# sailordiary/m3f.pytorch

Hardware: AMD Instinct MI355X
Metric: clips/sec (300-frame A+V, fwd+bwd) (higher is better)
Workload: dtype f32 (fp32-accurate products, fp32 accumulate: GEMMs as fp16x3 -- two fp16 terms per scaled operand, three MFMAs, error vs fp64 no larger than an fp32 GEMM's; the forward and backward recurrences at H=512 and H=256 as fp16x3 too (h is bounded; the backward producers split their values under a power-o

## Files before the change

include/m3t_hip.h:

```cpp
#ifndef M3T_HIP_H
#define M3T_HIP_H

#include <stddef.h>
#include <stdint.h>

#ifdef __cplusplus
extern "C" {
#endif

#define M3T_EINVAL 10001
#define M3T_MAX_SCANS 8
#define M3T_ESPIN 10002
#define M3T_SCAN_NO_PERSIST 1
#define M3T_SCAN_WHH 8
#define M3T_SCAN_FP32 4
#define M3T_SCAN_FAULT 16
#define M3T_SCAN_WIDE 32
#define M3T_BF16 2
#define M3T_GEMM_BACKGROUND 1
#define M3T_GEMM_BF16 2
#define M3T_GEMM_HIGH 256
#define M3T_GEMM_F16X3 1024
#define M3T_GEMM_BESIDE_SCAN 512
#define M3T_GEMM_EXCLUSIVE 8
// ... 105 lines not shown
    unsigned long long* amax;
    const float* wfrag;
} m3t_gru_bwd_desc;

size_t m3t_gru_bwd_prepare_floats(int H);
int m3t_gru_bwd_prepare(const float* const* w, int n, int H, int whh_direct, float* const* out, void* stream);

int m3t_gru_scan_workgroups(int n_scans, int H, int B, int T, int flags, int backward);
int m3t_gru_persist_count(void);
int m3t_gru_poll_error(void);
int m3t_gru_error_reset(void);
int m3t_gru_error_defer(int on);
int m3t_gru_inject_error(void* stream);
int m3t_gru_persist_owner(void);
int m3t_gru_scan_arena(void* arena, size_t bytes);
int m3t_gru_scan_arena_reset(void* arena);
int m3t_gru_scan_progress(unsigned* counters, int n_marks, const int* time_bounds, unsigned* need);
int m3t_gru_scan_progress_reset(unsigned* counters);
int m3t_gru_scan_progress_ok(int n_scans, int H, int B, int T, int flags, int backward);
int m3t_stream_wait_progress(const unsigned* counter, unsigned need, void* stream);
int m3t_gru_scan_after(void* event);
int m3t_gru_scan_events(void* start, void* end);
int m3t_gru_persist_profile(unsigned long long* out6);

int m3t_gru_scan_bwd(const m3t_gru_bwd_desc* scans, int n_scans, int B, int T,
                     float* ws, size_t ws_bytes, int flags, void* stream);

int m3t_att_fuse_fwd(const float* s_v, const float* s_a, const float* x_v, const float* x_a,
                     float* f, int rows, int D, void* stream);
int m3t_att_fuse_bwd(const float* df, const float* s_v, const float* s_a,
                     const float* x_v, const float* x_a,
                     float* ds_v, float* ds_a, float* dx_v, float* dx_a,
                     int rows, int D, void* stream);

int m3t_va_loss(const float* y_hat, int rows, int C, int iv, int ia,
                const float* valence, const float* arousal,
                const int64_t* class_expr, const uint8_t* expr_valid, int n_expr,
                float w_v, float w_a, float expr_w, int use_mse,
                float* out_scalars, float* dy, float* ws, size_t ws_bytes, void* stream);
size_t m3t_va_loss_ws_bytes(int rows);

size_t m3t_bn_cl_ws_bytes(size_t M, int C);
int m3t_bn_pool_cl_fwd(const float* x, size_t P, int H, int W, int C, int k, const float* gamma, const float* beta, float* run_mean, float* run_var,
                       float momentum, float eps, int training, float* yp, unsigned char* win, float* save_mean, float* save_invstd, float* ws,
                       size_t ws_bytes, void* stream);
int m3t_bn_pool_cl_bwd(const float* dyp, const float* x, const float* yp, const unsigned char* win, const float* gamma, const float* save_mean,
                       const float* save_invstd, size_t P, int H, int W, int C, int k, int training, float* dx, float* dgamma, float* dbeta,
                       float* dx_colsum, float* ws, size_t ws_bytes, void* stream);
int m3t_bn_cl_fwd(const float* x, size_t M, int C, const float* gamma, const float* beta, float* run_mean, float* run_var, float momentum,
                  float eps, int training, int relu, float* y, float* save_mean, float* save_invstd, float* ws, size_t ws_bytes, void* stream);
int m3t_bn_cl_bwd(const float* dy, const float* x, const float* y, const float* gamma, const float* save_mean, const float* save_invstd, size_t M,
                  int C, int training, int relu, float* dx, float* dgamma, float* dbeta, float* dx_colsum, float* ws, size_t ws_bytes, void* stream);
int m3t_pool_cl_fwd(const float* x, size_t P, int H, int W, int C, int kh, int kw, int sh, int sw, int ph, int pw, float* y, unsigned char* win,
                    void* stream);
int m3t_pool_cl_bwd(const float* dy, const unsigned char* win, size_t P, int H, int W, int C, int kh, int kw, int sh, int sw, int ph, int pw,
                    float* dx, void* stream);

int m3t_bn_add_relu_cl_fwd(const float* x, const float* shortcut, size_t M, int C, const float* gamma, const float* beta, float* run_mean,
                           float* run_var, float momentum, float eps, int training, float* y, float* save_mean, float* save_invstd, float* ws,
                           size_t ws_bytes, void* stream);
int m3t_bn_add_relu_cl_bwd(const float* dy, const float* x, const float* y, const float* gamma, const float* save_mean, const float* save_invstd,
                           size_t M, int C, int training, float* dx, float* ds, float* dgamma, float* dbeta, float* dx_colsum, float* ws,
                           size_t ws_bytes, void* stream);
int m3t_mean_cl_fwd(const float* x, size_t P, int HW, int C, float* y, void* stream);
int m3t_mean_cl_bwd(const float* dy, size_t P, int HW, int C, float* dx, void* stream);

// ... 260 lines not shown
```

m3f.pytorch_amd/csrc/fuse_loss.hip:

```cpp
#include "gru_common.h"
#include <cmath>
#include <cstdlib>
#include <mutex>

namespace {

__device__ __forceinline__ void fuse_weights(float sv, float sa, float& hv, float& ha, float& w0, float& w1) {
    hv = 1.f / (1.f + expf(-sv));
    ha = 1.f / (1.f + expf(-sa));
    const float m = fmaxf(hv, ha);
    const float ev = expf(hv - m), ea = expf(ha - m);
    const float inv = 1.f / (ev + ea);
    w0 = ev * inv;
    w1 = ea * inv;
}

__device__ __forceinline__ float mix2(float w0, float v, float w1, float a) { return fmaf(w0, v, w1 * a); }

__global__ __launch_bounds__(256) void att_fuse_fwd_kernel(const float* __restrict__ s_v, const float* __restrict__ s_a,
                                                           const float* __restrict__ x_v, const float* __restrict__ x_a,
                                                           float* __restrict__ f, int rows, int D, int vec) {
    const int lane = threadIdx.x & 63;
    const int row = blockIdx.x * 4 + (threadIdx.x >> 6);
    if (row >= rows) return;
// ... 23 lines not shown
    if (row >= rows) return;
    float hv, ha, w0, w1;
    fuse_weights(s_v[row], s_a[row], hv, ha, w0, w1);
    const size_t base = (size_t)row * D;
    float d0 = 0.f, d1 = 0.f;
    if (vec) {
        const float4* pg = reinterpret_cast<const float4*>(df + base);
        const float4* pv = reinterpret_cast<const float4*>(x_v + base);
        const float4* pa = reinterpret_cast<const float4*>(x_a + base);
        float4* qv = reinterpret_cast<float4*>(dx_v + base);
        float4* qa = reinterpret_cast<float4*>(dx_a + base);
        for (int i = lane; i < (D >> 2); i += 64) {
            const float4 g = pg[i], v = pv[i], a = pa[i];
            d0 += g.x * v.x + g.y * v.y + g.z * v.z + g.w * v.w;
            d1 += g.x * a.x + g.y * a.y + g.z * a.z + g.w * a.w;
            qv[i] = make_float4(w0 * g.x, w0 * g.y, w0 * g.z, w0 * g.w);
            qa[i] = make_float4(w1 * g.x, w1 * g.y, w1 * g.z, w1 * g.w);
        }
    } else {
        for (int i = lane; i < D; i += 64) {
            const float g = df[base + i];
            d0 += g * x_v[base + i];
            d1 += g * x_a[base + i];
            dx_v[base + i] = w0 * g;
            dx_a[base + i] = w1 * g;
        }
    }
    d0 = wave_sum(d0);
    d1 = wave_sum(d1);
    if (lane == 0) {
        const float dot = w0 * d0 + w1 * d1;
        ds_v[row] = w0 * (d0 - dot) * hv * (1.f - hv);
        ds_a[row] = w1 * (d1 - dot) * ha * (1.f - ha);
    }
}

__device__ __forceinline__ double wave_sum_d(double v) {
#pragma unroll
    for (int o = 32; o > 0; o >>= 1) v += __shfl_xor(v, o, 64);
    return v;
}
__device__ __forceinline__ double block_sum_d(double v, double* red) {
    const int lane = threadIdx.x & 63, w = threadIdx.x >> 6, nw = (blockDim.x + 63) >> 6;
    v = wave_sum_d(v);
    __syncthreads();
    if (lane == 0) red[w] = v;
    __syncthreads();
    double r = 0.0;
    for (int i = 0; i < nw; ++i) r += red[i];
    return r;
}

struct VaTerm { double mx, mt, ccc, mse, c1, c2, c3; };

__device__ __forceinline__ VaTerm va_term(double mx, double mt, double cov, double vsum, double mse, double invn, double nm1) {
    VaTerm s;
    const double den = vsum + (mx - mt) * (mx - mt);
    const double q = 2.0 * cov / (den * den);
    s.mx = mx; s.mt = mt; s.mse = mse;
    s.ccc = 2.0 * cov / den;
    s.c1 = 2.0 * invn / den;
    s.c2 = q * 2.0 * nm1;
    s.c3 = q * 2.0 * (mx - mt) * invn;
    return s;
}

// ... 387 lines not shown
extern "C" int m3t_sgd_step(float* p, const float* g, float* buf, size_t n, float lr, float momentum, float weight_decay,
                            int step, const float* guard, void* stream) {
    if (n == 0) return 0;
    if (!p || !g || !buf || step < 1) return M3T_EINVAL;
    int blocks = (int)((n + 255) / 256);
    if (blocks > 4096) blocks = 4096;
    sgd_kernel<<<blocks, 256, 0, (hipStream_t)stream>>>(p, g, buf, n, lr, momentum, weight_decay, step == 1, guard);
    M3T_LAUNCH_CHECK();
    return 0;
}

extern "C" int m3t_att_fuse_fwd(const float* s_v, const float* s_a, const float* x_v, const float* x_a, float* f,
                                int rows, int D, void* stream) {
    if (rows <= 0 || D <= 0) return 0;
    if (!s_v || !s_a || !x_v || !x_a || !f) return M3T_EINVAL;
    const int vec = (D % 4 == 0) && (((uintptr_t)x_v | (uintptr_t)x_a | (uintptr_t)f) % 16 == 0);
    att_fuse_fwd_kernel<<<cdiv(rows, 4), 256, 0, (hipStream_t)stream>>>(s_v, s_a, x_v, x_a, f, rows, D, vec);
    M3T_LAUNCH_CHECK();
    return 0;
}

extern "C" int m3t_att_fuse_bwd(const float* df, const float* s_v, const float* s_a, const float* x_v, const float* x_a,
                                float* ds_v, float* ds_a, float* dx_v, float* dx_a, int rows, int D, void* stream) {
    if (rows <= 0 || D <= 0) return 0;
    if (!df || !s_v || !s_a || !x_v || !x_a || !ds_v || !ds_a || !dx_v || !dx_a) return M3T_EINVAL;
    const int vec = (D % 4 == 0) &&
                    (((uintptr_t)x_v | (uintptr_t)x_a | (uintptr_t)df | (uintptr_t)dx_v | (uintptr_t)dx_a) % 16 == 0);
    att_fuse_bwd_kernel<<<cdiv(rows, 4), 256, 0, (hipStream_t)stream>>>(df, s_v, s_a, x_v, x_a, ds_v, ds_a, dx_v, dx_a,
                                                                         rows, D, vec);
    M3T_LAUNCH_CHECK();
    return 0;
}

extern "C" size_t m3t_va_loss_ws_bytes(int rows) { return rows > 0 ? (size_t)cdiv(rows, LB) * 16 * sizeof(double) : 0; }

extern "C" int m3t_va_loss(const float* y_hat, int rows, int C, int iv, int ia, const float* valence,
                           const float* arousal, const int64_t* class_expr, const uint8_t* expr_valid, int n_expr,
                           float w_v, float w_a, float expr_w, int use_mse, float* out_scalars, float* dy,
                           float* ws, size_t ws_bytes, void* stream) {
    if (rows <= 0 || C <= 0 || iv < 0 || ia < 0 || iv >= C || ia >= C || n_expr > C) return M3T_EINVAL;
    if (!y_hat || !valence || !arousal || !out_scalars || !dy) return M3T_EINVAL;
    if (n_expr > 0 && (!class_expr || !expr_valid)) return M3T_EINVAL;
    static const bool fused_on = !(getenv("M3T_VA_LOSS_FUSED") && getenv("M3T_VA_LOSS_FUSED")[0] == '0');
    const bool ws_ok = ws && ((uintptr_t)ws % 8) == 0 && ws_bytes >= m3t_va_loss_ws_bytes(rows);
    double* part = reinterpret_cast<double*>(ws);
    if (rows > 1024 && ws_ok && cdiv(rows, LB) <= 128 && fused_on) {
        VaSync* sync = va_sync_words();
        if (sync) {
            const int nb = cdiv(rows, LB);
            va_loss_fused_kernel<<<nb, LB, 0, (hipStream_t)stream>>>(y_hat, rows, C, iv, ia, valence, arousal, class_expr, expr_valid, n_expr, w_v,
                                                                     w_a, expr_w, use_mse, part, sync, 1 << 22, out_scalars, dy);
            M3T_LAUNCH_CHECK();
            return 0;
        }
    }
    if (rows > 1024 && ws_ok) {
        const int nb = cdiv(rows, LB);
        double* partA = part;
        double* partB = part + (size_t)nb * 8;
        hipStream_t s = (hipStream_t)stream;
        va_loss_sums_kernel<<<nb, LB, 0, s>>>(y_hat, rows, C, iv, ia, valence, arousal, class_expr, expr_valid, n_expr, partA);
        va_loss_moments_kernel<<<nb, LB, 0, s>>>(y_hat, rows, C, iv, ia, valence, arousal, partA, partB);
        va_loss_grad_kernel<<<nb, LB, 0, s>>>(y_hat, rows, C, iv, ia, valence, arousal, class_expr, expr_valid, n_expr, w_v, w_a,
                                             expr_w, use_mse, partA, partB, out_scalars, dy);
        M3T_LAUNCH_CHECK();
        return 0;
// ... 52 lines not shown
```

m3f.pytorch_amd/m3t/_lib.py:

```python
import ctypes as C
import os

_HERE = os.path.dirname(os.path.abspath(__file__))
LIB_PATH = os.environ.get("M3T_LIB_PATH") or os.path.join(os.path.dirname(_HERE), "lib", "libm3t_hip.so")
CSRC_DIR = os.path.join(os.path.dirname(_HERE), "csrc")

M3T_EINVAL = 10001
M3T_ESPIN = 10002
M3T_SCAN_NO_PERSIST = 1
M3T_BF16 = 2
M3T_GEMM_BESIDE_SCAN = 512
M3T_GEMM_F16X3 = 1024
M3T_GEMM_HIGH = 256
M3T_GEMM_EXCLUSIVE = 8
M3T_CONV_IMAGES = 4096
M3T_SCAN_FP32 = 4
M3T_SCAN_WHH = 8
M3T_SCAN_FAULT = 16
M3T_SCAN_WIDE = 32
M3T_MAX_SCANS = 8
M3T_JPEG_TRUNC, M3T_JPEG_CODE, M3T_JPEG_RST, M3T_JPEG_EXTRA = 1, 2, 4, 8

_f = C.c_void_p
_i = C.c_int
# ... 43 lines not shown
    "m3t_sgemm_bimg": [_i, _i, _i, _f, _i, _f, _f, _i, _f, _i, _i, _f, _z, _f, _f, _s],
    "m3t_sgemm_ring": [_i, _i, _i, _i, _i, _f, _i, _f, _i, _f, _i, _f, _i, _i, _i, _i, _i, _i, _f, _z, _i, _f, _f, _i, _s],
    "m3t_conv3d_taps_pre": [_f, _f, _f] + [_i] * 16 + [_f, _f, _f, _z, _f, _s],
    "m3t_conv3d_fwd_taps": [_f, _f, _f, _f] + [_i] * 15 + [_f, _f, _f, _z, _f, _s],
    "m3t_conv3d_fwd_taps4": [_f, _f, _f, _f] + [_i] * 14 + [_f, _f, _f, _z, _f, _s],
    "m3t_planes_to_cl4": [_f, _f, _i, _i, C.c_longlong, _s],
    "m3t_conv3d_wgrad_taps": [_f, _f, _f] + [_i] * 16 + [_f, _f, _f, _z, _s],
    "m3t_amax_out": [C.c_void_p],
    "m3t_colsum": [_f, _i, _i, _i, _f, _i, _f, _z, _s],
    "m3t_transpose": [_f, _i, _i, _i, _f, _i, _s],
    "m3t_relu_bwd": [_f, _f, _z, _s],
    "m3t_gru_scan_fwd": [C.POINTER(GruFwdDesc), _i, _i, _i, _f, _z, _i, _s],
    "m3t_gru_scan_bwd": [C.POINTER(GruBwdDesc), _i, _i, _i, _f, _z, _i, _s],
    "m3t_gru_bwd_prepare_floats": [_i],
    "m3t_gru_bwd_prepare": [C.POINTER(C.c_void_p), _i, _i, _i, C.POINTER(C.c_void_p), _s],
    "m3t_gru_persist_count": [],
    "m3t_gru_scan_workgroups": [_i, _i, _i, _i, _i, _i],
    "m3t_gru_poll_error": [],
    "m3t_gru_error_reset": [],
    "m3t_gru_error_defer": [_i],
    "m3t_gru_inject_error": [_s],
    "m3t_gru_persist_owner": [],
    "m3t_gru_scan_arena": [C.c_void_p, _z],
    "m3t_gru_scan_arena_reset": [C.c_void_p],
    "m3t_gru_scan_after": [C.c_void_p],
    "m3t_gru_scan_progress": [C.c_void_p, _i, C.POINTER(C.c_int), C.POINTER(C.c_uint)],
    "m3t_gru_scan_progress_reset": [C.c_void_p],
    "m3t_gru_scan_progress_ok": [_i, _i, _i, _i, _i, _i],
    "m3t_stream_wait_progress": [C.c_void_p, C.c_uint, _s],
    "m3t_gru_scan_events": [C.c_void_p, C.c_void_p],
    "m3t_gru_persist_profile": [C.c_void_p],
    "m3t_att_fuse_fwd": [_f, _f, _f, _f, _f, _i, _i, _s],
    "m3t_att_fuse_bwd": [_f, _f, _f, _f, _f, _f, _f, _f, _f, _i, _i, _s],
    "m3t_bn_cl_ws_bytes": [_z, _i],
    "m3t_bn_cl_fwd": [_f, _z, _i, _f, _f, _f, _f, C.c_float, C.c_float, _i, _i, _f, _f, _f, _f, _z, _s],
    "m3t_bn_cl_bwd": [_f, _f, _f, _f, _f, _f, _z, _i, _i, _i, _f, _f, _f, _f, _f, _z, _s],
    "m3t_bn_pool_cl_fwd": [_f, _z, _i, _i, _i, _i, _f, _f, _f, _f, C.c_float, C.c_float, _i, _f, C.c_void_p, _f, _f, _f, _z, _s],
    "m3t_bn_pool_cl_bwd": [_f, _f, _f, C.c_void_p, _f, _f, _f, _z, _i, _i, _i, _i, _i, _f, _f, _f, _f, _f, _z, _s],
    "m3t_pool_cl_fwd": [_f, _z, _i, _i, _i, _i, _i, _i, _i, _i, _i, _f, C.c_void_p, _s],
    "m3t_pool_cl_bwd": [_f, C.c_void_p, _z, _i, _i, _i, _i, _i, _i, _i, _i, _i, _f, _s],
    "m3t_bn_add_relu_cl_fwd": [_f, _f, _z, _i, _f, _f, _f, _f, C.c_float, C.c_float, _i, _f, _f, _f, _f, _z, _s],
    "m3t_bn_add_relu_cl_bwd": [_f, _f, _f, _f, _f, _f, _z, _i, _i, _f, _f, _f, _f, _f, _f, _z, _s],
    "m3t_mean_cl_fwd": [_f, _z, _i, _i, _f, _s],
    "m3t_mean_cl_bwd": [_f, _z, _i, _i, _f, _s],
    "m3t_gn_cl_ws_bytes": [_i, _z, _i],
    "m3t_gn_cl_fwd": [_f, _i, _z, _i, _i, _f, _f, C.c_float, _i, _f, _f, _f, _f, _z, _s],
    "m3t_gn_cl_bwd": [_f, _f, _f, _f, _f, _f, _i, _z, _i, _i, _i, _f, _f, _f, _f, _f, _z, _s],
    "m3t_gn_pool_cl_fwd": [_f, _i, _i, _i, _i, _i, _i, _i, _f, _f, C.c_float, _f, C.c_void_p, _f, _f, _f, _z, _s],
    "m3t_gn_pool_cl_bwd": [_f, _f, _f, C.c_void_p, _f, _f, _f, _i, _i, _i, _i, _i, _i, _i, _f, _f, _f, _f, _f, _z, _s],
    "m3t_relu_cl_ws_bytes": [_z, _i],
    "m3t_relu_cl_fwd": [_f, _z, _i, _f, _s],
    "m3t_relu_cl_bwd": [_f, _f, _z, _i, _f, _f, _f, _z, _s],
    "m3t_relu_pool_cl_fwd": [_f, _z, _i, _i, _i, _i, _f, C.c_void_p, _s],
    "m3t_relu_pool_cl_bwd": [_f, _f, C.c_void_p, _z, _i, _i, _i, _i, _f, _f, _f, _z, _s],
    "m3t_va_loss": [_f, _i, _i, _i, _i, _f, _f, _f, _f, _i, C.c_float, C.c_float, C.c_float, _i, _f, _f, _f, _z, _s],
    "m3t_va_loss_ws_bytes": [_i],
    "m3t_weight_norm_fwd": [_f, _f, _f, _f, _i, _i, _i, _s],
    "m3t_weight_norm_bwd": [_f, _f, _f, _f, _f, _f, _i, _i, _i, _s],
    "m3t_causal_conv_fwd": [_f, _f, _f, _f, _f, _f, _f, _i, _i, _i, _i, _i, _i, _i, _i, _s],
    "m3t_causal_conv_wgrad": [_f, _f, _f, _i, _i, _i, _i, _i, _i, _f, _z, _s],
    "m3t_conv1d_fwd": [_f, _f, _f, _f, _f, _f, _f, _i, _i, _i, _i, _i, _i, _i, _i, _i, C.c_float, C.c_ulonglong, _i, _s],
    "m3t_conv1d_fwd_scaled": [_f, _f, _f, _f, _f, _f, _f, _i, _i, _i, _i, _i, _i, _i, _i, _i, C.c_float, C.c_ulonglong, _i, _f, _f, _s],
    "m3t_conv1d_wgrad": [_f, _f, _f, _i, _i, _i, _i, _i, _i, _i, _f, _z, _i, _s],
    "m3t_conv1d_wgrad_scaled": [_f, _f, _f, _i, _i, _i, _i, _i, _i, _i, _f, _z, _i, _f, _f, _s],
    "m3t_pool_planes_fwd": [_f, C.c_longlong, _i, _i, _i, _i, _i, _i, _i, _i, _f, C.c_void_p, _s],
    "m3t_pool_planes_bwd": [_f, C.c_void_p, C.c_longlong, _i, _i, _i, _i, _i, _i, _i, _i, _f, _s],
# ... 133 lines not shown
```

m3f.pytorch_amd/m3t/ops.py:

```python
import ctypes as C
import os
import sys

import torch

from . import _lib
from ._lib import GruFwdDesc, GruBwdDesc, M3T_MAX_SCANS, M3THipError

_WS = {}
_WS_MIN = 64 << 20

PROFILE = []

import weakref

_GRAD_SINKS = {}


def register_grad_sink(param, view, owner=None):
    _GRAD_SINKS[id(param)] = [weakref.ref(param), view, False, id(owner) if owner is not None else None]


def clear_grad_sinks(owner=None):
    if owner is None:
# ... 874 lines not shown
    wgs = sum(2 * (Hs[i] // 16) * ((B + 15) // 16) for i in heavy)
    if light and wgs >= 192:
        return [("side", light), ("main", heavy)]
    return [("main", list(range(len(Hs))))]


def _interleaved(groups):
    return (_PERSIST_ENABLED and not SCAN_PER_STEP[0] and len(groups) == 2
            and all(kind == "main" for kind, _ in groups))


_CONCURRENT_ENABLED = os.environ.get("M3T_SCAN_CONCURRENT", "1") != "0"
_CUS = {}


def _pair_fits(dev, n_heavy, H_heavy, n_light, H_light, B, T, prec):
    if not _CONCURRENT_ENABLED:
        return False
    key = (dev.type, dev.index)
    cus = _CUS.get(key)
    if cus is None:
        cus = _CUS[key] = torch.cuda.get_device_properties(dev).multi_processor_count
    base = _scan_flags(dev) | prec
    if base & _lib.M3T_SCAN_NO_PERSIST:
        return False
    for bwd in (0, 1):
        a = lib().m3t_gru_scan_workgroups(n_heavy, H_heavy, B, T, base | _lib.M3T_SCAN_WIDE, bwd)
        b = lib().m3t_gru_scan_workgroups(n_light, H_light, B, T, base | _lib.M3T_SCAN_WIDE, bwd)
        if a <= 0 or b <= 0 or a + b > cus or (a + 7) // 8 + (b + 7) // 8 > cus // 8:
            return False
    return True


class _MultiBiGRU(torch.autograd.Function):

    @staticmethod
    def forward(ctx, n_stacks, L, cat_lo, cat_hi, unit_mask, *tensors):
        per = 1 + 8 * L
        assert len(tensors) == n_stacks * per
        xs, params = [], []
        for s in range(n_stacks):
            xs.append(_req(tensors[s * per].contiguous(), "x"))
            params.append([_req(t, "gru parameter") for t in tensors[s * per + 1:(s + 1) * per]])
        B, T = xs[0].shape[0], xs[0].shape[1]
        dev = xs[0].device
        for x in xs:
            if x.shape[0] != B or x.shape[1] != T:
                raise M3THipError("grouped GRU stacks must share batch and length")
        Hs = [params[s][1].shape[1] for s in range(n_stacks)]
        new = lambda *shape: torch.empty(*shape, dtype=torch.float32, device=dev)
        h_ns = [new(2 * L, B, Hs[s]) for s in range(n_stacks)]
        outs = [[new(B, T, 2 * Hs[s]) for s in range(n_stacks)] for _ in range(L)]
        cat_buf = None
        if cat_hi - cat_lo >= 2:
            cat_buf = new(B, T, sum(2 * Hs[s] for s in range(cat_lo, cat_hi)))
            off = 0
            for s in range(cat_lo, cat_hi):
                outs[L - 1][s] = cat_buf[..., off:off + 2 * Hs[s]]
                off += 2 * Hs[s]
        gates = [[new(2, B, T, 4 * Hs[s]) for s in range(n_stacks)] for _ in range(L)]
        xprojs = [[new(B, T, 6 * Hs[s]) for s in range(n_stacks)] for _ in range(L)]
        main = cur_stream()
        prec = _PREC[0]
        groups = _stream_groups(Hs, B)
        fslots = None
        if (prec & _lib.M3T_GEMM_F16X3) and all(h % 4 == 0 for h in Hs):
            fslots = amax_slots(n_stacks * (1 + 2 * L), dev)
            items = [(xs[s], fslots.data_ptr() + 8 * s) for s in range(n_stacks) if not (unit_mask >> s) & 1]
            wslot = {}
            ctx.w_keep = []
            for l in range(L):
                for s in range(n_stacks):
                    for d in (0, 1):
                        a = weight_amax(params[s][(2 * l + d) * 4], ctx.w_keep)
                        if a is None:
                            a = fslots.data_ptr() + 8 * (n_stacks + (l * n_stacks + s) * 2 + d)
                            items.append((params[s][(2 * l + d) * 4], a))
                        wslot[(l, s, d)] = a
            if not measure_amax(items):
                fslots = None
        one = amax_one(dev)

        def fslot_x(l, s):
            return None if fslots is None else (fslots.data_ptr() + 8 * s if (l == 0 and not (unit_mask >> s) & 1) else one)

        def fslot_w(l, s, d):
            return None if fslots is None else wslot[(l, s, d)]

        alone = not _interleaved(groups) and all(kind == "main" for kind, _ in groups)

        def level_fwd(l, idxs, scan, after=None, wide=False, progress=None):
            descs = []
            for s in idxs:
                H = Hs[s]
                inp = xs[s] if l == 0 else outs[l - 1][s]
                I = inp.shape[-1]
                for d in (0, 1):
                    w_ih, w_hh, b_ih, b_hh = params[s][(2 * l + d) * 4:(2 * l + d) * 4 + 4]
                    if not scan:
                        sgemm(0, 1, B * T, 3 * H, I, inp, 0, I, w_ih, 0, I, xprojs[l][s], d * 3 * H, 6 * H, bias=b_ih, prec=prec,
                              exclusive=alone, amax=(fslot_x(l, s), fslot_w(l, s, d)))
                    else:
                        descs.append(GruFwdDesc(_vp(xprojs[l][s]), _vp(w_hh), _vp(b_hh), _vp(outs[l][s]),
                                                _vp(gates[l][s], d * B * T * 4 * H), _vp(h_ns[s], (2 * l + d) * B * H),
                                                H, d, 6 * H, d * 3 * H, outs[l][s].stride(1), d * H))
            if scan:
                return _scan_fwd(descs, B, T, prec | (_lib.M3T_SCAN_WIDE if (wide or FORCE_WIDE_FWD[0]) else 0), after,
                                 None if progress is None else (_progress_counters(dev), progress))

        def chunk_plan(idxs, wide):
            if L < 2 or fslots is None or len({Hs[i] for i in idxs}) != 1 or 2 * len(idxs) > M3T_MAX_SCANS:
                return None
            H = Hs[idxs[0]]
            if H % 64 != 0:
                return None
            fl = _scan_flags(dev) | prec | (_lib.M3T_SCAN_WIDE if (wide or FORCE_WIDE_FWD[0]) else 0)
            if not lib().m3t_gru_scan_progress_ok(2 * len(idxs), H, B, T, fl, 0):
# ... 124 lines not shown
                if len({Hs[i] for i in idxs}) == 1 and H % 256 == 0 and 2 * len(idxs) <= M3T_MAX_SCANS \
                        and lib().m3t_gru_scan_progress_ok(2 * len(idxs), H, B, T, bfl, 1):
                    nfl = int(lib().m3t_gru_bwd_prepare_floats(H))
                    for l in range(L):
                        ws_, outs_ = [], []
                        for si in idxs:
                            for d in (0, 1):
                                buf = new(nfl)
                                wfq[(l, si, d)] = buf
                                ws_.append(params[si][(2 * l + d) * 4 + 1])
                                outs_.append(buf)
                        jobs.append((H, ws_, outs_))
            if jobs:
                wg1 = wgrad_streams(dev)[1]
                wg1.wait_stream(main)
                with on_stream(wg1):
                    for H, ws_, outs_ in jobs:
                        n_ = len(ws_)
                        _lib.check(lib().m3t_gru_bwd_prepare((C.c_void_p * n_)(*[t.data_ptr() for t in ws_]), n_, H, 1,
                                                             (C.c_void_p * n_)(*[t.data_ptr() for t in outs_]), _stream()), "m3t_gru_bwd_prepare")
                    ctx.wfq_ev = torch.cuda.Event()
                    ctx.wfq_ev.record(wg1)
                ctx.wfq = wfq
        ctx.n_stacks, ctx.L, ctx.Hs, ctx.B, ctx.T, ctx.prec = n_stacks, L, Hs, B, T, prec
        ctx.unit_mask = unit_mask
        ctx.concurrent = concurrent
        ctx.cat = (cat_lo, cat_hi) if cat_buf is not None else (0, 0)
        saved = []
        for l in range(L):
            for s in range(n_stacks):
                saved += [outs[l][s], gates[l][s]]
        ctx.has_fslots = fslots is not None
        ctx.wslot = wslot if fslots is not None else None
        if fslots is not None:
            for st_ in (side_stream(dev),):
                fslots.record_stream(st_)
            saved.append(fslots)
        ctx.save_for_backward(*(list(tensors) + saved))
        result = []
        for s in range(n_stacks):
            if cat_buf is not None and cat_lo <= s < cat_hi:
                result += [cat_buf if s == cat_lo else new(0), h_ns[s]]
            else:
                result += [outs[L - 1][s], h_ns[s]]
        return tuple(result)

    @staticmethod
    def backward(ctx, *grads):
        n_stacks, L, Hs, B, T = ctx.n_stacks, ctx.L, ctx.Hs, ctx.B, ctx.T
        per = 1 + 8 * L
        st = ctx.saved_tensors
        tensors, acts = st[:n_stacks * per], st[n_stacks * per:]
        fslots = None
        if ctx.has_fslots:
            fslots, acts = acts[-1], acts[:-1]
        params = [list(tensors[s * per + 1:(s + 1) * per]) for s in range(n_stacks)]
        xs = [tensors[s * per].contiguous() for s in range(n_stacks)]

        def layer_io(l, s):
            out, gts = acts[(l * n_stacks + s) * 2], acts[(l * n_stacks + s) * 2 + 1]
            inp = xs[s] if l == 0 else acts[((l - 1) * n_stacks + s) * 2]
            return inp, out, gts

        dev = params[0][0].device
        new = lambda *shape: torch.empty(*shape, dtype=torch.float32, device=dev)
        out_grads = [None] * (n_stacks * per)
        sunk = [False] * (n_stacks * per)
        douts, dhns = [], []
        cat_lo, cat_hi = ctx.cat
# ... 14 lines not shown
            dhns.append(None if gh is None else _req(gh.contiguous(), "dh_n"))
        dgx = [[new(B, T, 6 * Hs[s]) for s in range(n_stacks)] for _ in range(L)]
        dgh = [[new(2, B, T, 3 * Hs[s]) for s in range(n_stacks)] for _ in range(L)]
        dh = [[new(2, B, Hs[s]) for s in range(n_stacks)] for _ in range(L)]
        dbp = [[new(2, B, 4, Hs[s]) for s in range(n_stacks)] for _ in range(L)]
        direct_whh = all(h % 16 == 0 for h in Hs) and all(p.is_contiguous() for prm in params for p in prm)
        wht = [[[None if direct_whh else new(Hs[s], 3 * Hs[s]) for _ in (0, 1)] for s in range(n_stacks)] for _ in range(L)]
        need_dx = [[l > 0 or ctx.needs_input_grad[5 + s * per] for s in range(n_stacks)] for l in range(L)]
        dinp = [[torch.empty_like(layer_io(l, s)[0]) if need_dx[l][s] else None for s in range(n_stacks)] for l in range(L)]
        for s in range(n_stacks):
            for l in range(L):
                for d in (0, 1):
                    w_ih, w_hh = params[s][(2 * l + d) * 4], params[s][(2 * l + d) * 4 + 1]
                    base = s * per + 1 + (2 * l + d) * 4
                    for j, prm in enumerate(params[s][(2 * l + d) * 4:(2 * l + d) * 4 + 4]):
                        sink = _take_sink(prm)
                        out_grads[base + j] = sink if sink is not None else torch.empty_like(prm)
                        sunk[base + j] = sink is not None
        main = cur_stream()
        groups = _stream_groups(Hs, B)
        cur = {s: douts[s] for s in range(n_stacks)}
        prec = ctx.prec
        wfq = ctx.wfq or {}
        if ctx.wfq_ev is not None:
            main.wait_event(ctx.wfq_ev)
        NSL = _CHUNK_WINDOWS + 1
        bslots = amax_slots(2 * L * n_stacks * NSL, dev) if fslots is not None else None
        one = amax_one(dev)

        def bslot(l, s, d, j=-1):
            return None if bslots is None else bslots.data_ptr() + 8 * (((l * n_stacks + s) * 2 + d) * NSL + 1 + j)

        def fslot_x(l, s):
            return None if fslots is None else (fslots.data_ptr() + 8 * s if (l == 0 and not (ctx.unit_mask >> s) & 1) else one)

        def fslot_w(l, s, d):
            return None if fslots is None else ctx.wslot[(l, s, d)]

        def chunk_plan(l, idxs):
            if bslots is None or len({Hs[i] for i in idxs}) != 1 or 2 * len(idxs) > M3T_MAX_SCANS or not any(need_dx[l][s] for s in idxs):
                return None
            H = Hs[idxs[0]]
            if H % 64 != 0 or any(need_dx[l][s] and layer_io(l, s)[0].shape[-1] % 64 != 0 for s in idxs) or not direct_whh:
                return None
            fl = _scan_flags(dev) | prec | _lib.M3T_SCAN_WHH | _lib.M3T_SCAN_WIDE
            if not lib().m3t_gru_scan_progress_ok(2 * len(idxs), H, B, T, fl, 1):
                return None
            tb = _chunk_bounds(B, T, backward=True)
            return tb if (tb is not None and len(tb) + 1 <= _CHUNK_WINDOWS) else None

        def dx_pieces(l, idxs, tb, need, scan_stream):
            wg = wgs[1]
            ctr = _progress_counters(dev)
            ev_end = torch.cuda.Event()
            ev_end.record(scan_stream)
            lo, hi = [0] + tb, tb + [T]
            n = len(tb)
            with on_stream(wg):
                ended = False
                for dirn, k, w, second in _arrivals(tb, T):
                    if k is None:
                        if not ended:
                            wg.wait_event(ev_end)
                            ended = True
                    else:
                        _wait_progress(ctr, dirn, need[dirn * n + k])
                    d = 1 - dirn
# ... 184 lines not shown
                    ev_heavy = torch.cuda.Event()
                    ev_heavy.record(main)
                    level_gemms(l, heavy)
                    with on_stream(side):
                        level_scan(l, light, ev_heavy)
                        ev_light = torch.cuda.Event()
                        ev_light.record(side)
                        level_gemms(l, light)
            finally:
                _FENCED[0] = False
            main.wait_stream(side)
        else:
            for kind, idxs in groups:
                stream = main
                if kind == "side":
                    stream = side_stream(dev)
                    stream.wait_stream(main)
                with on_stream(stream):
                    for l in range(L - 1, -1, -1):
                        level_scan(l, idxs, progress=chunk_plan(l, idxs) if (kind == "main" and len(groups) == 1) else None)
                        level_gemms(l, idxs)
            for kind, _ in groups:
                if kind == "side":
                    main.wait_stream(side_stream(dev))
        for key_ in list(held):
            release_held(key_, None)
        weights_sunk = all(sunk[s * per + 1 + (2 * l + d) * 4 + j] for s in range(n_stacks) for l in range(L) for d in (0, 1) for j in (0, 1))
        if weights_sunk:
            for l in range(L):
                for s in range(n_stacks):
                    for t in (dgx[l][s], dgh[l][s]) + tuple(layer_io(l, s)[:2]):
                        for w_ in wgs:
                            t.record_stream(w_)
            for t in (bslots, fslots):
                if t is not None:
                    for w_ in wgs:
                        t.record_stream(w_)
            _WGRAD_PENDING[(dev.type, dev.index)] = True
        else:
            for w_ in wgs:
                main.wait_stream(w_)
        for s in range(n_stacks):
            out_grads[s * per] = dinp[0][s]
        return (None, None, None, None, None) + tuple(None if sunk[i] else g for i, g in enumerate(out_grads))


def multi_bigru(stacks, cat=None):
    L = stacks[0][2]
    flat = []
    for x, prm, l in stacks:
        if l != L:
            raise M3THipError("grouped GRU stacks must have the same depth")
        flat.append(x)
        flat.extend(prm)
    lo, hi = cat if cat is not None else (0, 0)
    unit_mask = sum(1 << i for i, (x, _, _) in enumerate(stacks) if _is_unit(x))
    res = _MultiBiGRU.apply(len(stacks), L, lo, hi, unit_mask, *flat)
    for i in range(len(stacks)):
        if res[2 * i].numel():
            res[2 * i]._m3t_unit = res[2 * i]._version + 1
    return [(res[2 * i], res[2 * i + 1]) for i in range(len(stacks))]


class _AttFuse(torch.autograd.Function):

    @staticmethod
    def forward(ctx, s_v, s_a, x_v, x_a):
        s_v, s_a = _req(s_v.contiguous(), "s_v"), _req(s_a.contiguous(), "s_a")
        x_v, x_a = _req(x_v.contiguous(), "x_v"), _req(x_a.contiguous(), "x_a")
        D = x_v.shape[-1]
        rows = x_v.numel() // D
        if x_a.shape != x_v.shape or s_v.numel() != rows or s_a.numel() != rows:
            raise M3THipError("att_fuse: shape mismatch")
        f = torch.empty_like(x_v)
        with _Timed("att_fuse_fwd_kernel", 1, 0, nbytes=4.0 * rows * (3 * D + 2)):
            _lib.check(lib().m3t_att_fuse_fwd(_p(s_v), _p(s_a), _p(x_v), _p(x_a), _p(f), rows, D, _stream()), "m3t_att_fuse_fwd")
        ctx.save_for_backward(s_v, s_a, x_v, x_a)
        return f

    @staticmethod
    def backward(ctx, df):
        s_v, s_a, x_v, x_a = ctx.saved_tensors
        df = _req(df.contiguous(), "df")
        D = x_v.shape[-1]
        rows = x_v.numel() // D
        ds_v, ds_a = torch.empty_like(s_v), torch.empty_like(s_a)
        dx_v, dx_a = torch.empty_like(x_v), torch.empty_like(x_a)
        with _Timed("att_fuse_bwd_kernel", 1, 0, nbytes=4.0 * rows * (5 * D + 4)):
            _lib.check(lib().m3t_att_fuse_bwd(_p(df), _p(s_v), _p(s_a), _p(x_v), _p(x_a), _p(ds_v), _p(ds_a), _p(dx_v),
                                              _p(dx_a), rows, D, _stream()), "m3t_att_fuse_bwd")
        return ds_v, ds_a, dx_v, dx_a


def att_fuse(s_v, s_a, x_v, x_a):
    return _AttFuse.apply(s_v, s_a, x_v, x_a)


class _VALoss(torch.autograd.Function):
    @staticmethod
    def forward(ctx, y_hat, valence, arousal, class_expr, expr_valid, iv, ia, n_expr, w_v, w_a, expr_w, use_mse):
        y = _req(y_hat.contiguous(), "y_hat")
        Cc = y.shape[-1]
        rows = y.numel() // Cc
        val = _req(valence.contiguous().float(), "valence")
        aro = _req(arousal.contiguous().float(), "arousal")
        cls = vld = None
        if n_expr > 0:
            cls = class_expr.contiguous().long()
            vld = expr_valid.contiguous().to(torch.uint8)
            if not cls.is_cuda or not vld.is_cuda:
                raise M3THipError("labels must be device tensors")
        stats = torch.empty(8, dtype=torch.float32, device=y.device)
        dy = torch.empty_like(y)
        ws = workspace(y.device)
        with _Timed("va_loss_kernels", 3, 0, nbytes=4.0 * rows * (3 * Cc + 3 * 2 + Cc) + (3.0 * rows * 9 if n_expr > 0 else 0.0)):
            rc = lib().m3t_va_loss(_p(y), rows, Cc, iv, ia, _p(val), _p(aro),
                                   C.c_void_p(cls.data_ptr()) if cls is not None else None,
                                   C.c_void_p(vld.data_ptr()) if vld is not None else None,
                                   n_expr, w_v, w_a, expr_w, int(use_mse), _p(stats), _p(dy), _p(ws), ws.numel() * 4, _stream())
        _lib.check(rc, "m3t_va_loss")
        ctx.save_for_backward(dy)
        ctx.mark_non_differentiable(stats)
        return stats[0], stats

    @staticmethod
    def backward(ctx, g_loss, g_stats):
        (dy,) = ctx.saved_tensors
        return (dy * g_loss,) + (None,) * 11
# ... 2319 lines not shown
```

m3f.pytorch_amd/models/att_fusion.py:

```python
import torch.nn as nn

from m3t import ops
from .rnn import GRU, run_grus


class AttFusion(nn.Module):
    def __init__(self, input_dim=[512, 512], hidden_dim=128):
        super().__init__()
        d_audio, d_video = input_dim[0], input_dim[1]
        self.use_proj = d_video != d_audio
        if self.use_proj:
            self.proj_v = nn.Linear(d_video, d_audio)
        self.scorer_a = GRU(d_audio, hidden_dim, 1, 1, 1)
        self.scorer_v = GRU(d_audio, hidden_dim, 1, 1, 1)

    def forward(self, x_a, x_v):
        if self.use_proj:
            x_v = ops.linear(x_v, self.proj_v.weight, self.proj_v.bias, 0)
        s_v, s_a = run_grus([self.scorer_v, self.scorer_a], [x_v, x_a])
        return ops.att_fuse(s_v, s_a, x_v, x_a)
```

Baseline: 2830.

## Fuse scorer head projection into attention-fusion kernels and reuse tagged input amax

Adds scored forward/backward kernels that compute the GRU scorer's linear head (dot of hidden state with fc weight plus bias) inside the attention-fusion kernel. In backward they emit dh directly, with the head's weight and bias gradients done through a small GEMM/colsum that can go on the wgrad stream. The forward kernel also computes the output amax for the fp16x3 path, and the GRU reuses a tagged input amax instead of recomputing it. This removes separate head-linear launches and amax passes, at the cost of more Python plumbing and a global handoff variable.

```diff
diff --git a/include/m3t_hip.h b/include/m3t_hip.h
--- a/include/m3t_hip.h
+++ b/include/m3t_hip.h
@@ -161,6 +161,13 @@
                      const float* x_v, const float* x_a,
                      float* ds_v, float* ds_a, float* dx_v, float* dx_a,
                      int rows, int D, void* stream);
+int m3t_att_fuse_scored_fwd(const float* h_v, const float* h_a, const float* w_v, const float* b_v,
+                            const float* w_a, const float* b_a, const float* x_v, const float* x_a,
+                            float* f, float* s_v, float* s_a, int rows, int W, int D, void* stream);
+int m3t_att_fuse_scored_bwd(const float* df, const float* s_v, const float* s_a,
+                            const float* x_v, const float* x_a, const float* w_v, const float* w_a,
+                            float* ds_v, float* ds_a, float* dx_v, float* dx_a, float* dh_v, float* dh_a,
+                            int rows, int W, int D, void* stream);
 
 int m3t_va_loss(const float* y_hat, int rows, int C, int iv, int ia,
                 const float* valence, const float* arousal,
diff --git a/m3f.pytorch_amd/csrc/fuse_loss.hip b/m3f.pytorch_amd/csrc/fuse_loss.hip
--- a/m3f.pytorch_amd/csrc/fuse_loss.hip
+++ b/m3f.pytorch_amd/csrc/fuse_loss.hip
@@ -79,6 +79,129 @@
         const float dot = w0 * d0 + w1 * d1;
         ds_v[row] = w0 * (d0 - dot) * hv * (1.f - hv);
         ds_a[row] = w1 * (d1 - dot) * ha * (1.f - ha);
+    }
+}
+
+__device__ __forceinline__ float head_score(const float* __restrict__ h, const float* __restrict__ w, int W, int lane) {
+    float acc = 0.f;
+    for (int i = lane; i < W; i += 64) acc = fmaf(h[i], w[i], acc);
+    return wave_sum(acc);
+}
+
+constexpr int SCORED_FWD_WAVES = 16;
+
+__global__ __launch_bounds__(64 * SCORED_FWD_WAVES) void att_fuse_scored_fwd_kernel(const float* __restrict__ h_v, const float* __restrict__ h_a,
+                                                                  const float* __restrict__ w_v, const float* __restrict__ w_a,
+                                                                  const float* __restrict__ b_v, const float* __restrict__ b_a,
+                                                                  const float* __restrict__ x_v, const float* __restrict__ x_a,
+                                                                  float* __restrict__ f, float* __restrict__ s_v,
+                                                                  float* __restrict__ s_a, int rows, int W, int D, int vec,
+                                                                  unsigned long long* __restrict__ slot) {
+    const int lane = threadIdx.x & 63;
+    const int row = blockIdx.x * SCORED_FWD_WAVES + (threadIdx.x >> 6);
+    float mx = 0.f;
+    if (row < rows) {
+        const float sv = head_score(h_v + (size_t)row * W, w_v, W, lane) + (b_v ? b_v[0] : 0.f);
+        const float sa = head_score(h_a + (size_t)row * W, w_a, W, lane) + (b_a ? b_a[0] : 0.f);
+        if (lane == 0) { s_v[row] = sv; s_a[row] = sa; }
+        float hv, ha, w0, w1;
+        fuse_weights(sv, sa, hv, ha, w0, w1);
+        const size_t base = (size_t)row * D;
+        if (vec) {
+            const float4* pv = reinterpret_cast<const float4*>(x_v + base);
+            const float4* pa = reinterpret_cast<const float4*>(x_a + base);
+            float4* pf = reinterpret_cast<float4*>(f + base);
+            for (int i = lane; i < (D >> 2); i += 64) {
+                const float4 v = pv[i], a = pa[i];
+                const float4 o = make_float4(mix2(w0, v.x, w1, a.x), mix2(w0, v.y, w1, a.y), mix2(w0, v.z, w1, a.z), mix2(w0, v.w, w1, a.w));
+                pf[i] = o;
+                mx = fmaxf(fmaxf(mx, m3t_fin_abs(o.x)), fmaxf(m3t_fin_abs(o.y), fmaxf(m3t_fin_abs(o.z), m3t_fin_abs(o.w))));
+            }
+        } else {
+            for (int i = lane; i < D; i += 64) {
+                const float o = mix2(w0, x_v[base + i], w1, x_a[base + i]);
+                f[base + i] = o;
+                mx = fmaxf(mx, m3t_fin_abs(o));
+            }
+        }
+    }
+    if (slot) {
+        __shared__ float red[SCORED_FWD_WAVES];
+        mx = wave_max(mx);
+        if (lane == 0) red[threadIdx.x >> 6] = mx;
+        __syncthreads();
+        if (threadIdx.x < 64) {
+            const float m = wave_max(threadIdx.x < SCORED_FWD_WAVES ? red[threadIdx.x] : 0.f);
+            const unsigned long long bits = (unsigned long long)__float_as_uint(m);
+            if (threadIdx.x == 0 && bits > __hip_atomic_load(slot, __ATOMIC_RELAXED, __HIP_MEMORY_SCOPE_AGENT)) atomicMax(slot, bits);
+        }
+    }
+}
+
+__device__ __forceinline__ float dot2_unfused(float w0, float d0, float w1, float d1) {
+#pragma clang fp contract(off)
+    return w0 * d0 + w1 * d1;
+}
+
+__global__ __launch_bounds__(256) void att_fuse_scored_bwd_kernel(const float* __restrict__ df, const float* __restrict__ s_v,
+                                                                  const float* __restrict__ s_a, const float* __restrict__ x_v,
+                                                                  const float* __restrict__ x_a, const float* __restrict__ w_v,
+                                                                  const float* __restrict__ w_a, float* __restrict__ ds_v,
+                                                                  float* __restrict__ ds_a, float* __restrict__ dx_v,
+                                                                  float* __restrict__ dx_a, float* __restrict__ dh_v,
+                                                                  float* __restrict__ dh_a, int rows, int W, int D, int vec,
+                                                                  int vecw) {
+    const int lane = threadIdx.x & 63;
+    const int row = blockIdx.x * 4 + (threadIdx.x >> 6);
+    if (row >= rows) return;
+    float hv, ha, w0, w1;
+    fuse_weights(s_v[row], s_a[row], hv, ha, w0, w1);
+    const size_t base = (size_t)row * D;
+    float d0 = 0.f, d1 = 0.f;
+    if (vec) {
+        const float4* pg = reinterpret_cast<const float4*>(df + base);
+        const float4* pv = reinterpret_cast<const float4*>(x_v + base);
+        const float4* pa = reinterpret_cast<const float4*>(x_a + base);
+        float4* qv = reinterpret_cast<float4*>(dx_v + base);
+        float4* qa = reinterpret_cast<float4*>(dx_a + base);
+        for (int i = lane; i < (D >> 2); i += 64) {
+            const float4 g = pg[i], v = pv[i], a = pa[i];
+            d0 += g.x * v.x + g.y * v.y + g.z * v.z + g.w * v.w;
+            d1 += g.x * a.x + g.y * a.y + g.z * a.z + g.w * a.w;
+            qv[i] = make_float4(w0 * g.x, w0 * g.y, w0 * g.z, w0 * g.w);
+            qa[i] = make_float4(w1 * g.x, w1 * g.y, w1 * g.z, w1 * g.w);
+        }
+    } else {
+        for (int i = lane; i < D; i += 64) {
+            const float g = df[base + i];
+            d0 += g * x_v[base + i];
+            d1 += g * x_a[base + i];
+            dx_v[base + i] = w0 * g;
+            dx_a[base + i] = w1 * g;
+        }
+    }
+    d0 = wave_sum(d0);
+    d1 = wave_sum(d1);
+    const float dot = dot2_unfused(w0, d0, w1, d1);
+    const float gv = w0 * (d0 - dot) * hv * (1.f - hv);
+    const float ga = w1 * (d1 - dot) * ha * (1.f - ha);
+    if (lane == 0) { ds_v[row] = gv; ds_a[row] = ga; }
+    const size_t hb = (size_t)row * W;
+    if (vecw) {
+        const float4* pwv = reinterpret_cast<const float4*>(w_v);
+        const float4* pwa = reinterpret_cast<const float4*>(w_a);
+        float4* qv = reinterpret_cast<float4*>(dh_v + hb);
+        float4* qa = reinterpret_cast<float4*>(dh_a + hb);
+        for (int i = lane; i < (W >> 2); i += 64) {
+            const float4 a = pwv[i], b = pwa[i];
+            qv[i] = make_float4(gv * a.x, gv * a.y, gv * a.z, gv * a.w);
+            qa[i] = make_float4(ga * b.x, ga * b.y, ga * b.z, ga * b.w);
+        }
+    } else {
+        for (int i = lane; i < W; i += 64) {
+            dh_v[hb + i] = gv * w_v[i];
+            dh_a[hb + i] = ga * w_a[i];
+        }
     }
 }
 
@@ -532,6 +655,34 @@
     return 0;
 }
 
+extern "C" int m3t_att_fuse_scored_fwd(const float* h_v, const float* h_a, const float* w_v, const float* b_v, const float* w_a,
+                                       const float* b_a, const float* x_v, const float* x_a, float* f, float* s_v, float* s_a,
+                                       int rows, int W, int D, void* stream) {
+    unsigned long long* slot = m3t_take_amax_out();
+    if (rows <= 0 || D <= 0) return 0;
+    if (W <= 0 || !h_v || !h_a || !w_v || !w_a || !x_v || !x_a || !f || !s_v || !s_a) return M3T_EINVAL;
+    const int vec = (D % 4 == 0) && (((uintptr_t)x_v | (uintptr_t)x_a | (uintptr_t)f) % 16 == 0);
+    att_fuse_scored_fwd_kernel<<<cdiv(rows, SCORED_FWD_WAVES), 64 * SCORED_FWD_WAVES, 0, (hipStream_t)stream>>>(
+        h_v, h_a, w_v, w_a, b_v, b_a, x_v, x_a, f, s_v, s_a, rows, W, D, vec, slot);
+    M3T_LAUNCH_CHECK();
+    return 0;
+}
+
+extern "C" int m3t_att_fuse_scored_bwd(const float* df, const float* s_v, const float* s_a, const float* x_v, const float* x_a,
+                                       const float* w_v, const float* w_a, float* ds_v, float* ds_a, float* dx_v, float* dx_a,
+                                       float* dh_v, float* dh_a, int rows, int W, int D, void* stream) {
+    if (rows <= 0 || D <= 0) return 0;
+    if (W <= 0 || !df || !s_v || !s_a || !x_v || !x_a || !w_v || !w_a || !ds_v || !ds_a || !dx_v || !dx_a || !dh_v || !dh_a)
+        return M3T_EINVAL;
+    const int vec = (D % 4 == 0) &&
+                    (((uintptr_t)x_v | (uintptr_t)x_a | (uintptr_t)df | (uintptr_t)dx_v | (uintptr_t)dx_a) % 16 == 0);
+    const int vecw = (W % 4 == 0) && (((uintptr_t)w_v | (uintptr_t)w_a | (uintptr_t)dh_v | (uintptr_t)dh_a) % 16 == 0);
+    att_fuse_scored_bwd_kernel<<<cdiv(rows, 4), 256, 0, (hipStream_t)stream>>>(df, s_v, s_a, x_v, x_a, w_v, w_a, ds_v, ds_a, dx_v,
+                                                                                dx_a, dh_v, dh_a, rows, W, D, vec, vecw);
+    M3T_LAUNCH_CHECK();
+    return 0;
+}
+
 extern "C" size_t m3t_va_loss_ws_bytes(int rows) { return rows > 0 ? (size_t)cdiv(rows, LB) * 16 * sizeof(double) : 0; }
 
 extern "C" int m3t_va_loss(const float* y_hat, int rows, int C, int iv, int ia, const float* valence,
diff --git a/m3f.pytorch_amd/m3t/_lib.py b/m3f.pytorch_amd/m3t/_lib.py
--- a/m3f.pytorch_amd/m3t/_lib.py
+++ b/m3f.pytorch_amd/m3t/_lib.py
@@ -99,6 +99,8 @@
     "m3t_gru_persist_profile": [C.c_void_p],
     "m3t_att_fuse_fwd": [_f, _f, _f, _f, _f, _i, _i, _s],
     "m3t_att_fuse_bwd": [_f, _f, _f, _f, _f, _f, _f, _f, _f, _i, _i, _s],
+    "m3t_att_fuse_scored_fwd": [_f, _f, _f, _f, _f, _f, _f, _f, _f, _f, _f, _i, _i, _i, _s],
+    "m3t_att_fuse_scored_bwd": [_f, _f, _f, _f, _f, _f, _f, _f, _f, _f, _f, _f, _f, _i, _i, _i, _s],
     "m3t_bn_cl_ws_bytes": [_z, _i],
     "m3t_bn_cl_fwd": [_f, _z, _i, _f, _f, _f, _f, C.c_float, C.c_float, _i, _i, _f, _f, _f, _f, _z, _s],
     "m3t_bn_cl_bwd": [_f, _f, _f, _f, _f, _f, _z, _i, _i, _i, _f, _f, _f, _f, _f, _z, _s],
diff --git a/m3f.pytorch_amd/m3t/ops.py b/m3f.pytorch_amd/m3t/ops.py
--- a/m3f.pytorch_amd/m3t/ops.py
+++ b/m3f.pytorch_amd/m3t/ops.py
@@ -930,6 +930,9 @@
     return True
 
 
+_GRU_X_EXT = [None]
+
+
 class _MultiBiGRU(torch.autograd.Function):
 
     @staticmethod
@@ -962,9 +965,11 @@
         prec = _PREC[0]
         groups = _stream_groups(Hs, B)
         fslots = None
+        x_ext = {s: t for s, t in enumerate(_GRU_X_EXT[0] or []) if t is not None and not (unit_mask >> s) & 1}
+        _GRU_X_EXT[0] = None
         if (prec & _lib.M3T_GEMM_F16X3) and all(h % 4 == 0 for h in Hs):
             fslots = amax_slots(n_stacks * (1 + 2 * L), dev)
-            items = [(xs[s], fslots.data_ptr() + 8 * s) for s in range(n_stacks) if not (unit_mask >> s) & 1]
+            items = [(xs[s], fslots.data_ptr() + 8 * s) for s in range(n_stacks) if not (unit_mask >> s) & 1 and s not in x_ext]
             wslot = {}
             ctx.w_keep = []
             for l in range(L):
@@ -980,7 +985,11 @@
         one = amax_one(dev)
 
         def fslot_x(l, s):
-            return None if fslots is None else (fslots.data_ptr() + 8 * s if (l == 0 and not (unit_mask >> s) & 1) else one)
+            if fslots is None:
+                return None
+            if l == 0 and s in x_ext:
+                return x_ext[s].data_ptr()
+            return fslots.data_ptr() + 8 * s if (l == 0 and not (unit_mask >> s) & 1) else one
 
         def fslot_w(l, s, d):
             return None if fslots is None else wslot[(l, s, d)]
@@ -1171,9 +1180,11 @@
                 saved += [outs[l][s], gates[l][s]]
         ctx.has_fslots = fslots is not None
         ctx.wslot = wslot if fslots is not None else None
+        ctx.x_ext = x_ext if fslots is not None else {}
         if fslots is not None:
             for st_ in (side_stream(dev),):
-                fslots.record_stream(st_)
+                for t_ in (fslots,) + tuple(x_ext.values()):
+                    t_.record_stream(st_)
             saved.append(fslots)
         ctx.save_for_backward(*(list(tensors) + saved))
         result = []
@@ -1254,7 +1265,11 @@
             return None if bslots is None else bslots.data_ptr() + 8 * (((l * n_stacks + s) * 2 + d) * NSL + 1 + j)
 
         def fslot_x(l, s):
-            return None if fslots is None else (fslots.data_ptr() + 8 * s if (l == 0 and not (ctx.unit_mask >> s) & 1) else one)
+            if fslots is None:
+                return None
+            if l == 0 and s in ctx.x_ext:
+                return ctx.x_ext[s].data_ptr()
+            return fslots.data_ptr() + 8 * s if (l == 0 and not (ctx.unit_mask >> s) & 1) else one
 
         def fslot_w(l, s, d):
             return None if fslots is None else ctx.wslot[(l, s, d)]
@@ -1505,7 +1520,7 @@
                     for t in (dgx[l][s], dgh[l][s]) + tuple(layer_io(l, s)[:2]):
                         for w_ in wgs:
                             t.record_stream(w_)
-            for t in (bslots, fslots):
+            for t in (bslots, fslots) + tuple(ctx.x_ext.values()):
                 if t is not None:
                     for w_ in wgs:
                         t.record_stream(w_)
@@ -1528,7 +1543,11 @@
         flat.extend(prm)
     lo, hi = cat if cat is not None else (0, 0)
     unit_mask = sum(1 << i for i, (x, _, _) in enumerate(stacks) if _is_unit(x))
-    res = _MultiBiGRU.apply(len(stacks), L, lo, hi, unit_mask, *flat)
+    _GRU_X_EXT[0] = [t if torch.is_tensor(t) else None for t in (_tagged_amax(x) if x.is_contiguous() else None for x, _, _ in stacks)]
+    try:
+        res = _MultiBiGRU.apply(len(stacks), L, lo, hi, unit_mask, *flat)
+    finally:
+        _GRU_X_EXT[0] = None
     for i in range(len(stacks)):
         if res[2 * i].numel():
             res[2 * i]._m3t_unit = res[2 * i]._version + 1
@@ -1567,6 +1586,109 @@
 
 def att_fuse(s_v, s_a, x_v, x_a):
     return _AttFuse.apply(s_v, s_a, x_v, x_a)
+
+
+ATT_FUSE_SCORED = [os.environ.get("M3T_ATT_FUSE_SCORED", "1") != "0"]
+
+
+def _head_wgrad(ds, h, w, b, need_w, need_b, prec):
+    W = h.shape[-1]
+    rows = h.numel() // W
+    dw = db = None
+    w_sink = _take_sink(w) if (need_w and id(w) in _GRAD_SINKS) else None
+    b_sink = _take_sink(b) if (need_b and b is not None and id(b) in _GRAD_SINKS) else None
+    if (need_w and id(w) in _GRAD_SINKS and w_sink is None) or (need_b and b is not None and id(b) in _GRAD_SINKS and b_sink is None):
+        join_wgrad(h.device)
+    wg = wgrad_stream(h.device, _LINEAR_RR[0]) if h.is_cuda else None
+    off = wg is not None and (w_sink is not None or b_sink is not None)
+    if off:
+        wg.wait_stream(cur_stream())
+    if need_w:
+        if w_sink is not None and off:
+            with on_stream(wg):
+                sgemm(1, 0, 1, W, rows, ds, 0, 1, h, 0, W, w_sink, 0, W, prec=prec)
+        else:
+            dw = w_sink if w_sink is not None else torch.empty_like(w)
+            sgemm(1, 0, 1, W, rows, ds, 0, 1, h, 0, W, dw, 0, W, prec=prec, exclusive=True)
+            if w_sink is not None:
+                dw = None
+    if need_b and b is not None:
+        if b_sink is not None and off:
+            with on_stream(wg):
+                colsum(ds, 0, rows, 1, 1, b_sink)
+        else:
+            db = b_sink if b_sink is not None else torch.empty(1, dtype=h.dtype, device=h.device)
+            colsum(ds, 0, rows, 1, 1, db)
+            if b_sink is not None:
+                db = None
+    if off:
+        ds.record_stream(wg)
+        h.record_stream(wg)
+        _WGRAD_PENDING[(h.device.type, h.device.index)] = True
+        _LINEAR_RR[0] += 1
+    return dw, db
+
+
+class _AttFuseScored(torch.autograd.Function):
+
+    @staticmethod
+    def forward(ctx, h_v, h_a, w_v, b_v, w_a, b_a, x_v, x_a):
+        ctx.params = (w_v, b_v, w_a, b_a)
+        h_v, h_a = _req(h_v.contiguous(), "h_v"), _req(h_a.contiguous(), "h_a")
+        x_v, x_a = _req(x_v.contiguous(), "x_v"), _req(x_a.contiguous(), "x_a")
+        w_v, w_a = _req(w_v.contiguous(), "w_v"), _req(w_a.contiguous(), "w_a")
+        D, W = x_v.shape[-1], h_v.shape[-1]
+        rows = x_v.numel() // D
+        if x_a.shape != x_v.shape or h_a.shape != h_v.shape or h_v.numel() != rows * W or w_v.numel() != W or w_a.numel() != W \
+                or (b_v is not None and b_v.numel() != 1) or (b_a is not None and b_a.numel() != 1):
+            raise M3THipError("att_fuse_scored: shape mismatch")
+        f = torch.empty_like(x_v)
+        s_v = torch.empty(x_v.shape[:-1] + (1,), dtype=x_v.dtype, device=x_v.device)
+        s_a = torch.empty_like(s_v)
+        slot = amax_slots(1, f.device) if (f.is_cuda and D % 4 == 0 and (_PREC[0] & _lib.M3T_GEMM_F16X3)) else None
+        if slot is not None:
+            amax_out(slot.data_ptr())
+        try:
+            with _Timed("att_fuse_fwd_kernel", 1, 0, nbytes=4.0 * (rows * (2 * W + 3 * D + 2) + 2 * W)):
+                _lib.check(lib().m3t_att_fuse_scored_fwd(_p(h_v), _p(h_a), _p(w_v), _p(b_v), _p(w_a), _p(b_a), _p(x_v), _p(x_a), _p(f),
+                                                         _p(s_v), _p(s_a), rows, W, D, _stream()), "m3t_att_fuse_scored_fwd")
+        except BaseException:
+            _amax_clear()
+            raise
+        _OUT_SLOT[0] = slot
+        ctx.save_for_backward(s_v, s_a, x_v, x_a, h_v, h_a, w_v, w_a)
+        ctx.prec = _PREC[0]
+        ctx.mark_non_differentiable(s_v, s_a)
+        ctx.set_materialize_grads(False)
+        return f, s_v, s_a
+
+    @staticmethod
+    def backward(ctx, df, _dsv, _dsa):
+        if df is None:
+            return (None,) * 8
+        s_v, s_a, x_v, x_a, h_v, h_a, w_v, w_a = ctx.saved_tensors
+        pw_v, pb_v, pw_a, pb_a = ctx.params
+        df = _req(df.contiguous(), "df")
+        D, W = x_v.shape[-1], h_v.shape[-1]
+        rows = x_v.numel() // D
+        ds_v, ds_a = torch.empty_like(s_v), torch.empty_like(s_a)
+        dx_v, dx_a = torch.empty_like(x_v), torch.empty_like(x_a)
+        dh_v, dh_a = torch.empty_like(h_v), torch.empty_like(h_a)
+        with _Timed("att_fuse_bwd_kernel", 1, 0, nbytes=4.0 * (rows * (5 * D + 2 * W + 4) + 2 * W)):
+            _lib.check(lib().m3t_att_fuse_scored_bwd(_p(df), _p(s_v), _p(s_a), _p(x_v), _p(x_a), _p(w_v), _p(w_a), _p(ds_v), _p(ds_a),
+                                                     _p(dx_v), _p(dx_a), _p(dh_v), _p(dh_a), rows, W, D, _stream()),
+                       "m3t_att_fuse_scored_bwd")
+        ni = ctx.needs_input_grad
+        dw_v, db_v = _head_wgrad(ds_v, h_v, pw_v, pb_v, ni[2], ni[3], ctx.prec)
+        dw_a, db_a = _head_wgrad(ds_a, h_a, pw_a, pb_a, ni[4], ni[5], ctx.prec)
+        return dh_v, dh_a, dw_v, db_v, dw_a, db_a, dx_v, dx_a
+
+
+def att_fuse_scored(h_v, h_a, w_v, b_v, w_a, b_a, x_v, x_a, return_scores=False):
+    _OUT_SLOT[0] = None
+    f, s_v, s_a = _AttFuseScored.apply(h_v, h_a, w_v, b_v, w_a, b_a, x_v, x_a)
+    f = _tag_out(f)
+    return (f, s_v, s_a) if return_scores else f
 
 
 class _VALoss(torch.autograd.Function):
diff --git a/m3f.pytorch_amd/models/att_fusion.py b/m3f.pytorch_amd/models/att_fusion.py
--- a/m3f.pytorch_amd/models/att_fusion.py
+++ b/m3f.pytorch_amd/models/att_fusion.py
@@ -17,5 +17,9 @@
     def forward(self, x_a, x_v):
         if self.use_proj:
             x_v = ops.linear(x_v, self.proj_v.weight, self.proj_v.bias, 0)
+        if ops.ATT_FUSE_SCORED[0] and isinstance(self.scorer_v.fc, nn.Linear) and isinstance(self.scorer_a.fc, nn.Linear):
+            (h_v, _), (h_a, _) = ops.multi_bigru([self.scorer_v.stack(x_v), self.scorer_a.stack(x_a)])
+            fv, fa = self.scorer_v.fc, self.scorer_a.fc
+            return ops.att_fuse_scored(h_v, h_a, fv.weight, fv.bias, fa.weight, fa.bias, x_v, x_a)
         s_v, s_a = run_grus([self.scorer_v, self.scorer_a], [x_v, x_a])
         return ops.att_fuse(s_v, s_a, x_v, x_a)
```

After: 2854 (median of 6 runs). No clear change (+0.8%).
